# WPI-MMR/gym_solo

Measured on AMD Instinct MI355X. Metric: env-steps/s (whole node), 4096 Solo8 envs/GPU, 1/2/4/8 MI355X, higher is better.
Workload: dtype f64

## Files before the change

### gym_solo_amd/csrc/solo_engine.hip

```cpp
#include <hip/hip_runtime.h>

#include <cstdio>
#include <cstdlib>
#include <cstring>
#include <new>
#include <string>
#include <vector>

#ifndef SOLO_F64_PAIR_BUILD
#define SOLO_F64_PAIR_BUILD 1
#endif
#include "solo_wave_ops.h"
#include "solo_pgs_gfx950.h"
#include "solo_step_kernel.h"
#include "solo_launch.h"

namespace solo_engine_detail {

struct EngineBase {
  virtual ~EngineBase() {}
  virtual int set_program(const SoloProgram* p) = 0;
  virtual int reset(const uint8_t* mask, hipStream_t s) = 0;
  virtual int settle(hipStream_t s) = 0;
  virtual int set_targets(const void* a, hipStream_t s) = 0;
// ... 273 lines not shown
    if (int rc = check_flags(flags)) return rc;
    HIP_TRY(hipSetDevice(device));
    return launch((const T*)a, flags, s);
  }

  static constexpr int kWavesPerSimd = solo::kWavesPerSimd<T>;
  int resident_robots() const {
    hipDeviceProp_t p;
    const int cus = (hipGetDeviceProperties(&p, device) == hipSuccess && p.multiProcessorCount > 0) ? p.multiProcessorCount : 256;
    return cus * 4 * kWavesPerSimd;
  }
  int resident_cache = 0;
  solo::PlanInput plan_input(int k, uint32_t flags) {
    if (resident_cache == 0) resident_cache = resident_robots();
    return {n, sizeof(T), resident_cache, cfg.steps_per_launch, cfg.rollout_streams, cfg.migrate_steps, ctl_active(), sensing, k, flags,
            settling ? 1 : decimation, state_terms, act_on, wrench_on};
  }
  Plan make_plan(int k, uint32_t flags) { return solo::make_plan(plan_input(k, flags)); }
  int ensure_scratch(const Plan& p, uint32_t flags) {
    const bool records = solo::leaves_records(flags);
    if (records && p.S > traj_steps) {
      HIP_TRY(hipDeviceSynchronize());
      if (traj) { (void)hipFree(traj); traj = nullptr; traj_steps = 0; }
      HIP_TRY(hipMalloc((void**)&traj, solo::record_reals(n, p.S) * sizeof(T)));
      traj_steps = p.S;
      if (contact_traj) { (void)hipFree(contact_traj); contact_traj = nullptr; }
    }
    if (sensing && records && contact_traj == nullptr && traj_steps > 0) {
      HIP_TRY(hipDeviceSynchronize());
      HIP_TRY(hipMalloc((void**)&contact_traj, solo::foot_force_reals(n, traj_steps) * sizeof(T)));
      hparams.contact_traj = contact_traj;
// ... 10 lines not shown
    return SOLO_OK;
  }

  Args rollout_args(const void* a, int k, uint32_t flags, void* obs_out, void* reward_out, void* done_out) const {
    return Args{(const T*)a, a ? (long long)n * SOLO_NUM_JOINTS : 0, k, flags, (flags & SOLO_STEP_OBS) ? (T*)obs_out : nullptr,
                (flags & SOLO_STEP_REWARD) ? (T*)reward_out : nullptr, (flags & SOLO_STEP_DONE) ? (uint8_t*)done_out : nullptr};
  }

  int rollout(const void* a, int k, uint32_t flags, void* obs_out, void* reward_out, void* done_out, hipStream_t s) override {
    if (int rc = check_fault()) return rc;
    if (int rc = check_flags(flags)) return rc;
    if (k == 0) return SOLO_OK;
    if (!a || k < 0) { err = "rollout needs actions [K][N][12]"; return SOLO_ERR_INVALID_ARG; }
    const Plan plan = make_plan(k, flags);
    const Args args = rollout_args(a, k, flags, obs_out, reward_out, done_out);
    if (int rc = rollout_impl(plan, args, s, nullptr, nullptr)) return rc;
    if (!solo::tail_needs_copy<T>(plan, k, flags)) return SOLO_OK;
    if (args.obs_out)
      HIP_TRY(hipMemcpyAsync(obs, args.obs_out + (size_t)(k - 1) * n * obs_dim, (size_t)n * obs_dim * sizeof(T), hipMemcpyDeviceToDevice, s));
    if (args.reward_out)
      HIP_TRY(hipMemcpyAsync(reward, args.reward_out + (size_t)(k - 1) * n, (size_t)n * sizeof(T), hipMemcpyDeviceToDevice, s));
    if (args.done_out)
      HIP_TRY(hipMemcpyAsync(done, args.done_out + (size_t)(k - 1) * n, (size_t)n, hipMemcpyDeviceToDevice, s));
    return SOLO_OK;
  }

  int rollout_impl(const Plan& plan, const Args& args, hipStream_t s, hipEvent_t* t0, hipEvent_t* t1) {
    HIP_TRY(hipSetDevice(device));
    const int groups = plan.slices;
    if (int rc = ensure_scratch(plan, args.flags)) return rc;
// ... 23 lines not shown
    return SOLO_OK;
  }

  int enqueue(const Plan& plan, const Args& args, const solo::EngineBuffers<T>& wired, const solo::Launch& l, bool resid, hipStream_t s) {
    solo::KBuffers<T> b;
    solo::QueueInit q;
    if (!solo::wire_launch(plan, args, wired, l, &b, &q)) {
      err = "internal error: the migration queue of a launch does not fit its slice's region";
      return SOLO_ERR_INVALID_ARG;
    }
    if (q.ints > 0) {
      launch_flat(solo::solo_queue_init_kernel, q.ints, s, q.q, q.ints, q.lo, q.count, q.rings, q.steps, q.chunk, q.order);
      HIP_TRY(hipGetLastError());
    }
    const solo::KParams<T>* params_dev = dparams;
    solo::with_step_kernel<T>(solo::choose_kernel(sensing, ctl_active(), settling, resid, b.queue != nullptr, args.flags, decimation, state_terms, act_on, wrench_on),
                              [&](solo::StepKernel<T> k) { hipLaunchKernelGGL(k, dim3(l.count), dim3(64), 0, s, params_dev, b); });
    HIP_TRY(hipGetLastError());
    return SOLO_OK;
  }

  hipStream_t sub[kMaxStreams] = {};
  hipEvent_t ev_fork = nullptr, ev_join[kMaxStreams] = {};
  int ensure_streams(int groups) {
    if (!ev_fork) HIP_TRY(hipEventCreateWithFlags(&ev_fork, hipEventDisableTiming));
    for (int g = 0; g < groups; ++g) {
      if (!sub[g]) HIP_TRY(hipStreamCreateWithFlags(&sub[g], hipStreamNonBlocking));
      if (!ev_join[g]) HIP_TRY(hipEventCreateWithFlags(&ev_join[g], hipEventDisableTiming));
    }
    return SOLO_OK;
  }
// ... 11 lines not shown
    for (int g = 0; g < plan.slices; ++g) {
      float t = 0;
      HIP_TRY(hipEventElapsedTime(&t, e0[g], e1[g]));
      total += t;
    }
    *ms = total / plan.slices / plan.launches;
    return SOLO_OK;
  }

  int time_step(const void* a, uint32_t flags, int reps, hipStream_t s, double* ms) override {
    if (int rc = check_flags(flags)) return rc;
    if (reps <= 0 || !ms) { err = "reps must be positive"; return SOLO_ERR_INVALID_ARG; }
    HIP_TRY(hipSetDevice(device));
    const int S = cfg.steps_per_launch > 1 ? cfg.steps_per_launch : 1;
    Plan plan = make_plan(reps * S, flags);
    if (cfg.steps_per_launch == -1) {
      plan.S = 1; plan.launches = reps; plan.migrate = 0;
      if (cfg.rollout_streams == -1) plan.slices = 1;
    }
    return timed(plan, rollout_args(a, reps * S, flags, nullptr, nullptr, nullptr), s, ms);
  }

  int time_rollout(const void* a, int k, uint32_t flags, void* obs_out, void* reward_out, void* done_out, hipStream_t s, double* ms) override {
    if (int rc = check_flags(flags)) return rc;
    if (k <= 0 || !ms) { err = "num_steps must be positive"; return SOLO_ERR_INVALID_ARG; }
    HIP_TRY(hipSetDevice(device));
    return timed(make_plan(k, flags), rollout_args(a, k, flags, obs_out, reward_out, done_out), s, ms);
  }

  int reserve(int k, uint32_t flags) override {
    if (k <= 0) { err = "num_steps must be positive"; return SOLO_ERR_INVALID_ARG; }
    if (int rc = check_flags(flags)) return rc;
    HIP_TRY(hipSetDevice(device));
    return solo::for_each_geometry(plan_input(k, flags), k, [&](const Plan& p) {
      if (int rc = ensure_scratch(p, flags)) return rc;
      return p.slices > 1 ? ensure_streams(p.slices) : (int)SOLO_OK;
    });
  }

  int plan(int k, SoloLaunchPlan* out) override {
    if (k <= 0 || !out) { err = "num_steps must be positive"; return SOLO_ERR_INVALID_ARG; }
// ... 204 lines not shown
      const std::vector<T> ones((size_t)n * SOLO_ACTUATOR_WIDTH, T(1));
      HIP_TRY(hipMalloc((void**)&act_ones, ones.size() * sizeof(T)));
      HIP_TRY(hipMemcpy(act_ones, ones.data(), ones.size() * sizeof(T), hipMemcpyHostToDevice));
    }
    if (wrench == nullptr) {
      HIP_TRY(hipMalloc((void**)&wrench, cnt * sizeof(T)));
      hparams.wrench = wrench;
      HIP_TRY(hipMemcpy(dparams, &hparams, sizeof(hparams), hipMemcpyHostToDevice));
    }
    if ((const void*)wrench != per_env) HIP_TRY(hipMemcpy(wrench, h.data(), cnt * sizeof(T), hipMemcpyHostToDevice));
    wrench_on = true;
    return point_actuators();
  }

  std::string name;
  const char* kernel_name() override {
    name = solo::kernel_name(solo::choose_kernel(sensing, ctl_active(), false, cfg.solver_residual_threshold > 0, false, SOLO_STEP_ALL, decimation, state_terms, act_on, wrench_on), sizeof(T));
    return name.c_str();
  }
};

EngineBase* make_engine_f64(const SoloConfig& cfg, const SoloModel& model, int32_t num_envs, int32_t device_id, int* rc);
#ifndef SOLO_TU_F32
EngineBase* make_engine_f64(const SoloConfig& cfg, const SoloModel& model, int32_t num_envs, int32_t device_id, int* rc) {
  auto* e = new (std::nothrow) Engine<double>();
  *rc = e ? e->init(cfg, model, num_envs, device_id) : (int)SOLO_ERR_HIP;
  return e;
}
#endif

}

// ... 162 lines not shown
```

### gym_solo_amd/csrc/solo_kernel_params.h

```cpp
#pragma once

#include <cmath>
#include <cstdint>
#include <cstring>
#include <string>

#include "../../include/solo_engine.h"

namespace solo {

enum RowType : int32_t { ROW_IDLE = 0, ROW_MOTOR = 1, ROW_NORMAL = 2, ROW_TAN1 = 3, ROW_TAN2 = 4, ROW_LIMIT = 5 };
enum BodyKind : int32_t { BODY_BASE = 0, BODY_UPPER = 1, BODY_LOWER = 2 };

__host__ __device__ constexpr int motor_lane(int dof) { return 16 * (dof >> 1) + (dof & 1); }
__host__ __device__ constexpr int sphere_lane(int s) { return 16 * (s >> 2) + 2 + 3 * (s & 3); }

__host__ __device__ constexpr int leg_sum_entry(int e) {
  constexpr int Z = 10, N = 32;
  constexpr int b[27] = {0, 3, 1, 4, 5, 2,
                         Z, 8, 7 | N, 9,
                         8 | N, Z, 6, Z, 9,
                         7, 6 | N, Z, Z, Z, 9,
                         11, 12, 13, 14, 15, 16};
  constexpr int i[27] = {0, 1, 1, 2, 2, 2, 3, 3, 3, 3, 4, 4, 4, 4, 4, 5, 5, 5, 5, 5, 5, 0, 1, 2, 3, 4, 5};
// ... 129 lines not shown
  int32_t* term_count;
  double* stats;
  const T* terrain;
  const int32_t* order;
  int32_t* cost;
  T* warm;
  int32_t num_envs;
  uint32_t flags;
  int32_t env_base;
  int32_t count;
  int32_t steps;
  long long action_stride, done_stride;
  int32_t* queue;
  int32_t q_rings, q_chunk;
  int32_t* fault;
#ifdef SOLO_STAMPS
  int32_t stamp_row;
  unsigned long long* stamps;
  unsigned long long* acc;
#endif
};

inline int validate_model(const SoloModel& m, std::string* err) {
  auto fail = [&](const char* s) { if (err) *err = s; return (int)SOLO_ERR_UNSUPPORTED_MODEL; };
  for (int leg = 0; leg < 4; ++leg) {
    if (m.parent[2 * leg] != 0) return fail("HFE link must hang off the base");
    if (m.parent[2 * leg + 1] != 1 + 2 * leg) return fail("KFE link must hang off its HFE link");
  }
  for (int j = 0; j < SOLO_NUM_DOF; ++j)
    if (m.joint_axis[j][0] != 0.0 || m.joint_axis[j][1] != 1.0 || m.joint_axis[j][2] != 0.0)
// ... 165 lines not shown
```

### gym_solo_amd/csrc/solo_launch.h

```cpp
#pragma once

#include <string>

#include "solo_kernel_params.h"

namespace solo {

constexpr int kMaxStreams = 8;

struct Plan { int S, launches, slices, migrate; };

struct PlanInput {
  int n;
  size_t real_bytes;
  int resident;
  int32_t steps_per_launch, rollout_streams, migrate_steps;
  bool ctl_active, sensing;
  int k;
  uint32_t flags;
  int decimation = 1;
  bool state_terms = false;
  bool actuators = false;
  bool wrench = false;
};

inline Plan make_plan(const PlanInput& in) {
  const int n = in.n, k = in.k;
  const uint32_t flags = in.flags;
  const long long cap = ((1ll << 32) - 1) / ((long long)n * SOLO_STATE_STRIDE);
  const int decim = in.decimation > 1 ? in.decimation : 1;
  const int S_auto = 250 / decim > 1 ? 250 / decim : 1;
  long long want = in.steps_per_launch == -1 ? (k < S_auto ? k : S_auto) : (in.steps_per_launch > 1 ? in.steps_per_launch : 1);
  if (want > k && k > 0) want = k;
  Plan p;
  p.S = (int)(want < cap ? want : (cap > 1 ? cap : 1));
  if (p.S < 1) p.S = 1;
  p.launches = (k + p.S - 1) / p.S;
  const bool physics_only = flags == SOLO_STEP_PHYSICS;
  int streams = in.rollout_streams == -1 ? (p.launches > 1 ? 2 : 1) : in.rollout_streams;
  streams = streams < 1 ? 1 : (streams > kMaxStreams ? kMaxStreams : streams);
  p.migrate = 0;
#ifndef SOLO_STAMPS
  if (decim > 1 || in.state_terms || in.actuators || in.wrench) p.migrate = 0;
  else if (in.migrate_steps > 0) p.migrate = in.migrate_steps;
  else if (in.migrate_steps == -1 && !physics_only && (flags & SOLO_STEP_PHYSICS) && p.S >= 8 && !in.ctl_active && !in.sensing) {
    if (n > in.resident && in.real_bytes == 8) {
      if (p.launches == 1) p.migrate = (p.S + 1) / 2;
      else if (p.S >= 50) { p.migrate = 25; if (in.rollout_streams == -1) streams = 1; }
    }
  }
#endif
  p.slices = (streams > 1 && n >= 2 * streams) ? streams : 1;
  return p;
}

inline int max_slices(int n, int32_t rollout_streams) {
  const int streams = rollout_streams == -1 ? 2 : (rollout_streams < 1 ? 1 : (rollout_streams > kMaxStreams ? kMaxStreams : rollout_streams));
  return (streams > 1 && n >= 2 * streams) ? streams : 1;
}

inline int slice_begin(int n, int g, int groups) { return (int)((long long)n * g / groups); }

inline int queue_slots_per_robot(const Plan& p) {
  const int chunks = migration_chunks(p.S, p.migrate);
  return 1 + (chunks < 127 ? chunks : 127);
}

inline bool leaves_records(uint32_t flags) { return (flags & (SOLO_STEP_OBS | SOLO_STEP_REWARD)) != 0; }
inline size_t record_reals(int n, int steps) { return (size_t)steps * (size_t)n * SOLO_STATE_STRIDE; }
inline size_t foot_force_reals(int n, int steps) { return (size_t)steps * (size_t)n * 4; }
inline size_t queue_ints(int n, const Plan& p) {
  return p.migrate > 0 ? (size_t)kMaxStreams * kQueueHeader + (size_t)n * (size_t)queue_slots_per_robot(p) : 0;
}

template <class F>
inline int for_each_geometry(PlanInput in, int k, F&& f) {
  int last_S = -1, last_m = -1;
  for (int kk = 1; kk <= k; kk = (kk < 512 ? kk + 1 : (kk * 2 < k ? kk * 2 : (kk == k ? k + 1 : k)))) {
    in.k = kk;
    const Plan p = make_plan(in);
    if (p.S == last_S && p.migrate == last_m) continue;
    last_S = p.S; last_m = p.migrate;
    if (int rc = f(p)) return rc;
  }
  return 0;
}

enum KernelFamily : int { KERNEL_STEP = 0, KERNEL_CTL = 1, KERNEL_CONTACT = 2, KERNEL_DECIM = 3, KERNEL_TERM = 4, KERNEL_ACT = 5, KERNEL_PUSH = 6 };
struct KernelId {
  KernelFamily family;
  bool full, resid, migrate, ctl;
};

inline KernelId choose_kernel(bool sensing, bool ctl_active, bool settling, bool resid, bool has_queue, uint32_t flags, int decimation = 1,
                              bool state_terms = false, bool actuators = false, bool wrench = false) {
  const bool full = flags != SOLO_STEP_PHYSICS;
  if (wrench && !settling && (flags & SOLO_STEP_PHYSICS)) return {KERNEL_PUSH, full, false, false, ctl_active};
  if (actuators && !settling && ((flags & SOLO_STEP_PHYSICS) || (state_terms && (flags & SOLO_STEP_DONE)))) return {KERNEL_ACT, full, false, false, ctl_active};
  if (state_terms && !settling && (flags & (SOLO_STEP_PHYSICS | SOLO_STEP_DONE))) return {KERNEL_TERM, full, false, false, ctl_active};
  if (decimation > 1 && !settling && (flags & SOLO_STEP_PHYSICS)) return {KERNEL_DECIM, full, false, false, ctl_active};
  if (sensing && !settling) return {KERNEL_CONTACT, full, false, false, ctl_active};
  if (ctl_active && !settling) return {KERNEL_CTL, full, false, false, true};
  if (has_queue) return {KERNEL_STEP, true, resid, true, false};
  return {KERNEL_STEP, full, resid, false, false};
}

inline std::string kernel_name(const KernelId& id, size_t real_bytes) {
  const auto b = [](bool v) { return v ? ", true" : ", false"; };
  const std::string real = real_bytes == 4 ? "float" : "double";
  switch (id.family) {
    case KERNEL_CONTACT: return "solo_contact_kernel<" + real + b(id.full) + b(id.ctl) + ">";
    case KERNEL_CTL: return "solo_ctl_step_kernel<" + real + b(id.full) + ">";
    case KERNEL_DECIM: return "solo_decim_kernel<" + real + b(id.full) + b(id.ctl) + ">";
    case KERNEL_TERM: return "solo_term_kernel<" + real + b(id.full) + b(id.ctl) + ">";
    case KERNEL_ACT: return "solo_act_kernel<" + real + b(id.full) + b(id.ctl) + ">";
    case KERNEL_PUSH: return "solo_push_kernel<" + real + b(id.full) + b(id.ctl) + ">";
    default: return "solo_step_kernel<" + real + b(id.full) + b(id.resid) + b(id.migrate) + ">";
  }
}

template <typename T>
using StepKernel = void (*)(const KParams<T>*, KBuffers<T>);

template <typename T, class F>
inline void with_step_kernel(const KernelId& id, F&& f) {
  StepKernel<T> k;
  if (id.family == KERNEL_CONTACT) {
    if (id.ctl) k = !id.full ? solo_contact_kernel<T, false, true> : solo_contact_kernel<T, true, true>;
    else k = !id.full ? solo_contact_kernel<T, false, false> : solo_contact_kernel<T, true, false>;
  } else if (id.family == KERNEL_DECIM) {
    if (id.ctl) k = !id.full ? solo_decim_kernel<T, false, true> : solo_decim_kernel<T, true, true>;
    else k = !id.full ? solo_decim_kernel<T, false, false> : solo_decim_kernel<T, true, false>;
  } else if (id.family == KERNEL_TERM) {
    if (id.ctl) k = !id.full ? solo_term_kernel<T, false, true> : solo_term_kernel<T, true, true>;
    else k = !id.full ? solo_term_kernel<T, false, false> : solo_term_kernel<T, true, false>;
  } else if (id.family == KERNEL_ACT) {
    if (id.ctl) k = !id.full ? solo_act_kernel<T, false, true> : solo_act_kernel<T, true, true>;
    else k = !id.full ? solo_act_kernel<T, false, false> : solo_act_kernel<T, true, false>;
  } else if (id.family == KERNEL_PUSH) {
    if (id.ctl) k = !id.full ? solo_push_kernel<T, false, true> : solo_push_kernel<T, true, true>;
    else k = !id.full ? solo_push_kernel<T, false, false> : solo_push_kernel<T, true, false>;
  } else if (id.family == KERNEL_CTL) {
    k = !id.full ? solo_ctl_step_kernel<T, false> : solo_ctl_step_kernel<T, true>;
  } else if (id.migrate) {
    k = id.resid ? solo_step_kernel<T, true, true, true> : solo_step_kernel<T, true, false, true>;
  } else if (!id.full) {
    k = id.resid ? solo_step_kernel<T, false, true> : solo_step_kernel<T, false, false>;
  } else {
    k = id.resid ? solo_step_kernel<T, true, true> : solo_step_kernel<T, true, false>;
  }
  f(k);
}

template <typename T>
struct EngineBuffers {
  T *state, *snapshot, *targets, *params;
  T *obs, *reward;
  uint8_t* done;
// ... 17 lines not shown
template <typename T>
struct RolloutArgs {
  const T* act;
  long long act_stride;
  int k;
  uint32_t flags;
  T *obs_out, *reward_out;
  uint8_t* done_out;
};

struct Launch {
  int i, steps, lo, count, slice;
  bool final_chunk;
};

template <class F>
inline int for_each_launch(const Plan& plan, int n, int k, F&& f) {
  const int S = plan.S, groups = plan.slices;
  for (int i = 0; i < k; i += S)
    for (int g = 0; g < groups; ++g) {
      const int lo = slice_begin(n, g, groups), hi = slice_begin(n, g + 1, groups);
      if (int rc = f(Launch{i, (k - i < S) ? (k - i) : S, lo, hi - lo, g, i + S >= k})) return rc;
    }
  return 0;
}

struct QueueInit {
  int32_t* q;
  size_t ints;
  int lo, count, rings, steps, chunk;
  const int32_t* order;
};

template <typename T>
inline bool wire_launch(const Plan& plan, const RolloutArgs<T>& a, const EngineBuffers<T>& e, const Launch& l, KBuffers<T>* out, QueueInit* qi) {
  const int n = e.n, i = l.i, steps = l.steps;
  const uint32_t flags = a.flags;
  KBuffers<T>& b = *out;
  b.state = e.state; b.snapshot = e.snapshot; b.targets = e.targets; b.actions = a.act ? a.act + (size_t)i * a.act_stride : nullptr;
  b.params = e.params; b.traj = nullptr; b.obs_inline = b.reward_inline = nullptr; b.done = e.done; b.term_count = e.term_count;
  b.obs_rec = b.reward_rec = b.view_obs = b.view_reward = nullptr; b.view_done = nullptr; b.obs_rec_stride = b.reward_rec_stride = 0; b.obs_from = 0;
  b.stats = e.stats; b.terrain = e.terrain; b.order = e.order; b.cost = e.cost; b.num_envs = n; b.flags = flags;
  b.env_base = l.lo; b.count = l.count; b.steps = steps;
  b.action_stride = a.act_stride; b.done_stride = 0;
  b.queue = nullptr; b.q_rings = 1; b.q_chunk = 0;
  b.fault = e.fault;
  b.warm = e.warm;
#ifdef SOLO_STAMPS
  b.stamps = e.stamps;
#endif
  if (a.done_out) { b.done = a.done_out + (size_t)i * n; b.done_stride = n; }
  const bool want_obs = (flags & SOLO_STEP_OBS) != 0, want_reward = (flags & SOLO_STEP_REWARD) != 0;
  const bool inline_outputs = steps == 1 && (want_obs || want_reward) && kInlineOutputs<T, true>;
  if (inline_outputs) {
    if (want_obs) b.obs_inline = a.obs_out ? a.obs_out + (size_t)i * n * e.obs_dim : e.obs;
    if (want_reward) b.reward_inline = a.reward_out ? a.reward_out + (size_t)i * n : e.reward;
  } else if (want_obs || want_reward) {
    b.traj = e.traj + (size_t)l.lo * (size_t)e.traj_steps * SOLO_STATE_STRIDE;
    const bool tail_to_view = l.final_chunk;
    if (want_obs) {
      if (a.obs_out) { b.obs_rec = a.obs_out + (size_t)i * n * e.obs_dim; b.obs_rec_stride = (long long)n * e.obs_dim; if (tail_to_view) b.view_obs = e.obs; }
      else b.view_obs = e.obs;
// ... 9 lines not shown
    const int chunk = migration_chunk_steps(steps, plan.migrate);
    b.q_chunk = chunk;
    b.q_rings = migration_rings(l.count);
    b.queue = e.queue + (size_t)l.slice * kQueueHeader + (size_t)l.lo * (size_t)queue_slots_per_robot(plan);
    const size_t ints = migration_queue_ints(l.count, steps, chunk);
    if (ints > (size_t)kQueueHeader + (size_t)l.count * (size_t)queue_slots_per_robot(plan) ||
        (size_t)(b.queue - e.queue) + ints > e.queue_len)
      return false;
    *qi = QueueInit{b.queue, ints, l.lo, l.count, b.q_rings, steps, chunk, e.order};
  }
  return true;
}

template <typename T>
inline bool tail_needs_copy(const Plan& plan, int k, uint32_t flags) {
  const int last_steps = (k % plan.S == 0) ? plan.S : k % plan.S;
  return !leaves_records(flags) || (last_steps == 1 && kInlineOutputs<T, true>);
}

template <typename T>
inline void pack_control(const SoloConfig& cfg, const SoloControl& c, KParams<T>* P) {
  CtlConst<T>& k = P->ctl;
  k.mode = c.mode;
  for (int d = 0; d < SOLO_NUM_DOF; ++d) { k.kp[d] = (T)c.kp[d]; k.kd[d] = (T)c.kd[d]; }
  k.action_scale = (T)(c.mode == SOLO_CTRL_POSITION ? cfg.action_scale : c.action_scale);
  for (int j = 0; j < SOLO_NUM_JOINTS; ++j) k.reset_cmd[j] = (T)(c.mode == SOLO_CTRL_TORQUE ? 0.0 : cfg.settle_targets[j]);
}

template <typename T>
inline int validate_actuators(const T* host, int n, std::string* err) {
  for (size_t i = 0; i < (size_t)n * SOLO_ACTUATOR_WIDTH; ++i)
// ... 44 lines not shown
```

### gym_solo_amd/csrc/solo_step_body.h

```cpp
#pragma once

namespace solo {

template <typename T, bool kFull, bool kResid, bool kMigrate, bool kCtl, bool kContact, bool kDecim, bool kTerms, bool kAct = false, bool kPush = false>
__device__ __forceinline__ void step_body(const KParams<T>* Pin, const KBuffers<T>& Bin) {
  static_assert(!kTerms || kDecim, "the termination kernels run the substep loop");
  static_assert(!kAct || (kTerms && !kContact && !kResid && !kMigrate), "the actuator kernels are termination kernels: slot 25 of s_leg is theirs, and no robot migrates");
  static_assert(!kPush || kAct, "the push kernels are actuator kernels: their body plus the wrench");
  KBuffers<T> B = Bin;
  if (!kFull) B.flags = SOLO_STEP_PHYSICS;
  using R = Real<T>;
  __shared__ T s_state[SOLO_STATE_STRIDE];
  constexpr int kRS = ColumnBank<T>::kRowStride;
  constexpr int kRowsReals = kRowBlockReals<T>;
  constexpr int kGeoRows = SOLO_MAX_SPHERES + 1;
  __shared__ T s_blk[kRowsReals + kGeoRows * 4];
  static_assert(kRowsReals >= SOLO_MAX_REWARD_OPS * (kRowsReals / SOLO_MAX_REWARD_OPS < 32 ? kRowsReals / SOLO_MAX_REWARD_OPS : 32), "the output epilogue's scratch");
  T* const s_rowvec = s_blk;
  T (*const s_hext)[8] = ColumnBank<T>::kCompact ? nullptr : reinterpret_cast<T (*)[8]>(s_blk + 64 * kRS);
  __shared__ unsigned char s_rowleg[64];
  T (*const s_rowgeo)[4] = reinterpret_cast<T (*)[4]>(s_blk + kRowsReals);
  __shared__ int32_t s_rowtype[64];
  __shared__ T s_keep[32];
  __shared__ T s_leg[4][kLegSlots];
// ... 17 lines not shown
#pragma unroll
    for (int t = 0; t < SOLO_MAX_TERMS; ++t) r = r || solo_term_kind_reads_state(s_termtick[t]);
    return r;
  };
  const int lane0 = lane_id();
  const int slot = block_id() + B.env_base;
  if (slot >= B.num_envs) return;
  if (wave_cold_args(Bin)->num_envs != B.num_envs || wave_cold_args(Bin)->steps != B.steps) __builtin_trap();
  const int32_t* order = wave_cold_args(Bin)->order;
  int32_t* const queue = kMigrate ? wave_cold_args(Bin)->queue : nullptr;
  int env = 0, step_begin = 0, step_end = B.steps;
  bool last_chunk = true;
  int q_ring = 0, q_rings_left = 0, q_sweeps = 0, q_chunk_at = 0;
  int next_ticket = 0;
  bool have_next = false;
  if constexpr (!kMigrate) env = order != nullptr ? wave_uniform(order[slot]) : B.env_base + xcd_contiguous(block_id(), B.count);
  else {
    const int per_xcd = B.q_rings >= 8 ? B.q_rings >> 3 : 1;
    q_ring = B.q_rings >= 8 ? (wave_xcc_id() & 7) * per_xcd + (block_id() >> 3) % per_xcd : 0;
    q_rings_left = B.q_rings;
  }
#ifdef SOLO_STAMPS
  B.stamp_row = env;
#ifndef SOLO_STAMPS_LIGHT
  __shared__ unsigned long long s_acc[17];
  if (lane0 < 17) s_acc[lane0] = lane0 == 16 ? __builtin_amdgcn_s_memtime() : 0ull;
  B.acc = s_acc;
  wave_sync();
#endif
#endif
// ... 81 lines not shown
      if (ready >= 0) break;
      wave_backoff();
    }
    if (ready < 0) {
      if (lane0 == 0) { stats_add(&wave_cold_args(Bin)->stats[6], 1.0); if (wave_cold_args(Bin)->fault != nullptr) wave_fault_set(wave_cold_args(Bin)->fault); }
      break;
    }
    wave_acquire_device();
    env = B.env_base + (ready & 0xffffff);
    q_chunk_at = ready >> 24;
    step_begin = q_chunk_at * B.q_chunk;
    step_end = step_begin + B.q_chunk < B.steps ? step_begin + B.q_chunk : B.steps;
    last_chunk = step_end == B.steps;
  }
  const size_t rec = (size_t)env * SOLO_STATE_STRIDE;
  if constexpr (!ColumnBank<T>::kCompact) {
#pragma unroll
    for (int i = 0; i < 8; ++i) s_hext[lane0][i] = T(0);
  }
  if constexpr (!kMigrate) load_tables();
  T state_w = T(0);
  int count_w = 0;
  if constexpr (kMigrate) {
    if (lane0 < SOLO_STATE_STRIDE) state_w = wave_load_shared(wave_cold_args(Bin)->state + rec + lane0);
    if (lane0 < SOLO_MAX_TERMS) count_w = wave_atomic_load(wave_cold_args(Bin)->term_count + (size_t)env * SOLO_MAX_TERMS + lane0);
  } else {
    if (lane0 < SOLO_STATE_STRIDE) state_w = wave_cold_args(Bin)->state[rec + lane0];
    if (lane0 < SOLO_MAX_TERMS) count_w = wave_cold_args(Bin)->term_count[(size_t)env * SOLO_MAX_TERMS + lane0];
  }
  T foot_w = T(0);
  if constexpr (kContact) { if (lane0 < 4) foot_w = P0->contact[((size_t)env * SOLO_MAX_SPHERES + 4 * lane0 + 1) * SOLO_CONTACT_WIDTH + 3]; }
  const T mu = wave_cold_args(Bin)->params[(size_t)env * 4 + 0];
  const T mass_scale = wave_cold_args(Bin)->params[(size_t)env * 4 + 1];
  const T mu_base = P0->mu_base;
  T act_w = T(1);
  if constexpr (kAct) { if (lane0 < 3) act_w = P0->actuators[(size_t)env * SOLO_ACTUATOR_WIDTH + lane0]; }
  int hist_w = 0, prio_steps = 0;
  int prio_unit = 1;
  if constexpr (kDecim) prio_unit = wave_uniform(P0->decimation);
  if (B.steps == 1) {
    const int32_t* cost = wave_cold_args(Bin)->cost;
    if ((B.flags & SOLO_STEP_PHYSICS) && cost != nullptr) { hist_w = cost[env]; prio_steps = prio_unit; }
  }
  if constexpr (kMigrate) {
    if (lane0 == 0) hist_w = wave_atomic_load(queue + kQueueHeader + (env - B.env_base));
    hist_w = wave_readlane_int(hist_w, 0);
    prio_steps = step_begin;
  }
  {
    if constexpr (!kMigrate) store_tables();
    if (lane0 < SOLO_STATE_STRIDE) s_state[lane0] = state_w;
    if (lane0 < SOLO_MAX_TERMS) s_cnt[lane0] = count_w;
    if constexpr (sizeof(T) == 8) { if (lane0 == 0) { s_keep[27] = mu; s_keep[28] = mass_scale; } }
    if (lane0 == 0) s_keep[29] = mu_base;
    if constexpr (kContact) { if (lane0 < 4) s_leg[lane0][25] = foot_w; }
    if constexpr (kAct) {
      if (lane0 < 2) s_keep[30 + lane0] = act_w;
      const T act_kd = wave_readlane(act_w, SOLO_ACT_KD);
      if (lane0 < 4) s_leg[lane0][25] = act_kd;
    }
  }
  int prio_sweeps = wave_uniform(hist_w);
  const int hist_sweeps = kMigrate ? 0 : prio_sweeps;
  int prio_rot = (prio_steps + wave_slot_id()) % 3;
  if (prio_steps > 0) wave_set_priority_level(prio_sweeps > kPrioSweeps<T> * (kMigrate ? prio_steps : prio_unit) ? 3 : wave_slot_id() % 3);
  wave_sync();
  if constexpr (!kMigrate) make_term_tables();
  const bool may_restart = (B.flags & SOLO_STEP_DONE) && (B.flags & (SOLO_STEP_PHYSICS | SOLO_STEP_AUTO_RESET)) &&
                           wave_uniform(s_const.auto_reset) != 0;

  wave_sync();
#pragma unroll 1
  for (int step = step_begin; step < step_end; ++step) {
    const StepConst<T>& C = s_const;
    constexpr bool kLean = sizeof(T) == 8;
    int lane = kLean ? wave_fresh_lane() : wave_opaque_lane(lane0);
    const bool have_actions = kLean ? wave_opaque_bits((unsigned long long)B.actions) != 0ull : B.actions != nullptr;
    const T* const actions = have_actions ? B.actions : nullptr;
    const StepTables<T> tabs = {s_legc, s_rowtype, s_rowgeo};
    bool motor_lane = (s_rowtype[lane] & 15) == ROW_MOTOR;
    auto fetch_target = [&](int ln) -> T {
      const size_t tgt_at = (size_t)env * SOLO_NUM_JOINTS + (size_t)(3 * (ln >> 4) + (ln & 15));
// ... 118 lines not shown
        if (rt == ROW_TAN2) {
          T* const out = P0->contact + ((size_t)env * SOLO_MAX_SPHERES + sph) * SOLO_CONTACT_WIDTH;
          const T zr = T(wave_opaque_lane(0));
          out[0] = zr; out[1] = zr; out[2] = zr; out[3] = zr;
          if ((sph & 3) == 1) s_leg[sph >> 2][25] = zr;
        }
      }
      wave_sync();
      if (B.traj != nullptr && lane < 4)
        P0->contact_traj[((size_t)env * P0->contact_traj_steps + step) * 4 + lane] = s_leg[lane][25];
    }
    if (B.traj != nullptr) {
      const T ev = T((done ? kEventDone : 0) | (restart ? kEventRestart : 0) | fired_bits);
      const T word = s_state[lane & (SOLO_STATE_STRIDE - 1)];
      if (lane < SOLO_STATE_STRIDE)
        B.traj[(unsigned)((env - B.env_base) * B.steps + step) * (unsigned)SOLO_STATE_STRIDE + (unsigned)lane] = lane == SOLO_S_SPARE ? ev : word;
    }
    if constexpr (kInlineOutputs<T, kFull>) if (B.obs_inline != nullptr || B.reward_inline != nullptr) {
      const int n_obs = wave_uniform(C.num_obs), n_rops = wave_uniform(C.num_reward_ops);
      const ObsElemK<T> prog_obs = P0->obs[lane < n_obs ? lane : 0];
      const RewardInstrK<T> prog_reward = P0->reward[lane < n_rops ? lane : 0];
      const T angle = euler_component<T>(lane < 3 ? lane : 0, s_state[SOLO_S_QUAT], s_state[SOLO_S_QUAT + 1], s_state[SOLO_S_QUAT + 2], s_state[SOLO_S_QUAT + 3]);
      const T roll = wave_readlane(angle, 0), pitch = wave_readlane(angle, 1), yaw = wave_readlane(angle, 2);
      if (B.obs_inline != nullptr && lane < n_obs) {
        if constexpr (kContact) B.obs_inline[(size_t)env * n_obs + lane] = observation_value_foot<T>(prog_obs, s_state, roll, pitch, yaw, &s_leg[0][25], kLegSlots);
        else B.obs_inline[(size_t)env * n_obs + lane] = observation_value<T>(prog_obs, s_state, roll, pitch, yaw);
      }
      if (B.reward_inline != nullptr) {
        const RewardInstrK<T>& ri = prog_reward;
        T myval = reward_is_leaf(ri.op) ? reward_leaf<T>(ri, s_state, roll, pitch) : T(0);
        for (int i = 0; i < n_rops; ++i) {
// ... 35 lines not shown
    }
    SOLO_STAMP(B, 12);
    wave_sync();
  }
  SOLO_STAMP(B, 13);
  const int lane1 = sizeof(T) == 8 ? wave_fresh_lane() : wave_opaque_lane(lane0);
  if constexpr (kFull) if (B.traj != nullptr) {
    wave_fence_global();
    SOLO_STAMP_E(B, 1);
    const auto A = wave_cold_args(Bin);
    const int n_obs = wave_uniform(s_const.num_obs), n_rops = wave_uniform(s_const.num_reward_ops);
    constexpr int kPass = kRowsReals / SOLO_MAX_REWARD_OPS < 32 ? kRowsReals / SOLO_MAX_REWARD_OPS : 32;
    static_assert(kPass >= 16 && sizeof(T) * 32 >= (size_t)kPass, "the output epilogue's scratch");
    T* const val = s_blk;
    uint8_t* const ev_bytes = reinterpret_cast<uint8_t*>(s_keep);
    const T* const my_traj = B.traj + (size_t)(env - B.env_base) * (size_t)B.steps * SOLO_STATE_STRIDE;
    const bool want_reward = (B.flags & SOLO_STEP_REWARD) != 0;
    const bool bookkeeping = want_reward && (B.flags & SOLO_STEP_DONE) != 0;
    T* const obs_rec = A->obs_rec; T* const reward_rec = A->reward_rec;
    T* const view_obs = A->view_obs; T* const view_reward = A->view_reward; uint8_t* const view_done = A->view_done;
    const long long obs_stride = A->obs_rec_stride, reward_stride = A->reward_rec_stride;
    const int obs_from = A->obs_from;
    for (int base = step_begin; base < step_end; base += kPass) {
      const int k = base + lane1;
      if (lane1 < kPass && k < step_end) {
        const T* rec = my_traj + (size_t)k * SOLO_STATE_STRIDE;
        const bool last = k == B.steps - 1;
        const int ev = (int)rec[SOLO_S_SPARE];
        ev_bytes[lane1] = (uint8_t)ev;
        if (B.flags & SOLO_STEP_DONE) {
          if (B.done_stride != 0 || last) B.done[(size_t)k * B.done_stride + env] = (uint8_t)(ev & kEventDone);
          if (view_done != nullptr && last) view_done[env] = (uint8_t)(ev & kEventDone);
          if constexpr (kTerms) { if (last && (!kAct || state_program())) P0->term_fired[env] = (uint8_t)(ev >> 2); }
        }
        SOLO_STAMP_E(B, 2);
        T roll, pitch, yaw;
        euler_from_quat<T>(rec[SOLO_S_QUAT], rec[SOLO_S_QUAT + 1], rec[SOLO_S_QUAT + 2], rec[SOLO_S_QUAT + 3], &roll, &pitch, &yaw);
        SOLO_STAMP_E(B, 3);
        if (B.flags & SOLO_STEP_OBS) {
          T* o_rec = (obs_rec != nullptr && k >= obs_from) ? obs_rec + (size_t)k * obs_stride + (size_t)env * n_obs : nullptr;
          T* o_view = (view_obs != nullptr && last) ? view_obs + (size_t)env * n_obs : nullptr;
// ... 13 lines not shown
          if (view_reward != nullptr && last) view_reward[env] = rv;
        }
        SOLO_STAMP_E(B, 5);
      }
      wave_sync();
      SOLO_STAMP_E(B, 6);
      if (bookkeeping && lane1 == 0) {
        const int cnt = step_end - base < kPass ? step_end - base : kPass;
        accumulate_returns<T>(s_state, ev_bytes, 1, val + (size_t)(n_rops - 1) * kPass, 1, cnt, SOLO_STATS_ROW,
                              [](double* p, double x) { stats_add(p, x); });
      }
      wave_sync();
      SOLO_STAMP_E(B, 7);
    }
  }
  if ((B.flags & SOLO_STEP_DONE) && lane1 < SOLO_MAX_TERMS) {
    if constexpr (kMigrate) wave_atomic_store(wave_cold_args(Bin)->term_count + (size_t)env * SOLO_MAX_TERMS + lane1, s_cnt[lane1]);
    else wave_cold_args(Bin)->term_count[(size_t)env * SOLO_MAX_TERMS + lane1] = s_cnt[lane1];
  }
  if ((B.flags & SOLO_STEP_PHYSICS) && lane1 == 0 && last_chunk) { int32_t* cost = wave_cold_args(Bin)->cost; if (cost != nullptr) cost[env] = prio_sweeps - hist_sweeps; }
  const bool own_returns = (B.flags & SOLO_STEP_REWARD) && (B.flags & SOLO_STEP_DONE) &&
                           (B.traj != nullptr || (kInlineOutputs<T, kFull> && B.reward_inline != nullptr));
  if (lane1 < (own_returns ? SOLO_S_SPARE : SOLO_S_RETURN)) {
    if constexpr (kMigrate) wave_store_shared(wave_cold_args(Bin)->state + rec + lane1, s_state[lane1]);
    else wave_cold_args(Bin)->state[rec + lane1] = s_state[lane1];
  }
  SOLO_STAMP(B, 14);
#if defined(SOLO_STAMPS) && !defined(SOLO_STAMPS_LIGHT)
  wave_sync();
  if (lane1 < 16) B.stamps[(size_t)env * 32 + 16 + lane1] = s_acc[lane1];
#endif
  if constexpr (kMigrate) {
    const int chunks = migration_chunks(B.steps, B.q_chunk), ring_len = (B.count / B.q_rings) * chunks;
    int at = 0, nt = 0;
    if (lane1 == 0) {
      if (!last_chunk) {
        wave_atomic_store(queue + kQueueHeader + (env - B.env_base), prio_sweeps);
        at = wave_atomic_add(queue + q_ring * 32 + 16, 1);
      }
      nt = wave_atomic_add(queue + q_ring * 32, 1);
    }
    wave_release_device();
    if (!last_chunk && lane1 == 0)
      wave_atomic_store(queue + kQueueHeader + (size_t)B.count + (size_t)q_ring * ring_len + at, (env - B.env_base) | ((q_chunk_at + 1) << 24));
    next_ticket = wave_readlane_int(nt, 0);
    have_next = true;
  }
  if constexpr (kMigrate) wave_sync();
  } while (kMigrate);
#undef SOLO_STATS_ROW
}

}
```

### gym_solo_amd/csrc/solo_step_kernel.h

```cpp
#pragma once

#include "solo_kernel_params.h"
#include "solo_outputs.h"

#if defined(SOLO_STAMPS) && defined(SOLO_STAMPS_LIGHT)
#define SOLO_STAMP(B, i)                                                                          \
  do {                                                                                            \
    if (((i) == 0 || (i) == 14) && solo::lane_id() == 0)                                          \
      (B).stamps[(size_t)(B).stamp_row * 32 + (i)] = __builtin_amdgcn_s_memrealtime();         \
  } while (0)
#elif defined(SOLO_STAMPS)
#ifdef SOLO_STAMPS_EPILOGUE
#define SOLO_STAMP_ON(i) ((i) == 0 || (i) >= 13)
#define SOLO_STAMP_E(B, i) SOLO_STAMP_AT(B, i)
#else
#define SOLO_STAMP_ON(i) true
#endif
#define SOLO_STAMP(B, i) do { if (SOLO_STAMP_ON(i)) SOLO_STAMP_AT(B, i); } while (0)
#define SOLO_STAMP_AT(B, i)                                                                       \
  do {                                                                                            \
    if (solo::lane_id() == 0) {                                                                   \
      const unsigned long long t_ = __builtin_amdgcn_s_memtime();                                 \
      (B).stamps[(size_t)(B).stamp_row * 32 + (i)] = t_;                                            \
      (B).acc[(i)] += t_ - (B).acc[16];                                                           \
// ... 958 lines not shown
__global__ __launch_bounds__(64, kWavesPerSimd<T>) void solo_term_kernel(const KParams<T>* __restrict__ Pin, KBuffers<T> Bin) {
  step_body<T, kFull, false, false, kCtl, false, true, true>(Pin, Bin);
}

template <typename T, bool kFull, bool kCtl>
__global__ __launch_bounds__(64, kWavesPerSimd<T>) void solo_act_kernel(const KParams<T>* __restrict__ Pin, KBuffers<T> Bin) {
  step_body<T, kFull, false, false, kCtl, false, true, true, true>(Pin, Bin);
}

template <typename T, bool kFull, bool kCtl>
__global__ __launch_bounds__(64, kWavesPerSimd<T>) void solo_push_kernel(const KParams<T>* __restrict__ Pin, KBuffers<T> Bin) {
  step_body<T, kFull, false, false, kCtl, false, true, true, true, true>(Pin, Bin);
}

template <typename T>
__global__ void solo_contact_zero_kernel(T* __restrict__ contact, const uint8_t* __restrict__ mask, int num_envs) {
  const int i = blockIdx.x * blockDim.x + threadIdx.x;
  const int env = i / (SOLO_MAX_SPHERES * SOLO_CONTACT_WIDTH);
  if (env >= num_envs) return;
  if (mask != nullptr && mask[env] == 0) return;
  contact[i] = T(0);
}

static __global__ void solo_queue_init_kernel(int32_t* __restrict__ q, size_t ints, int env_base, int n, int rings, int steps, int chunk,
                                       const int32_t* __restrict__ order) {
  const size_t i = (size_t)blockIdx.x * blockDim.x + threadIdx.x;
  if (i < ints) migration_queue_init(q, i, env_base, n, rings, steps, chunk, order);
}

template <typename T>
// ... 43 lines not shown
```

Before: 200.0 million.

## Fuse multiple rollout launches into one segmented roll kernel

```diff
diff --git a/gym_solo_amd/csrc/solo_engine.hip b/gym_solo_amd/csrc/solo_engine.hip
--- a/gym_solo_amd/csrc/solo_engine.hip
+++ b/gym_solo_amd/csrc/solo_engine.hip
@@ -311,7 +311,7 @@
   solo::PlanInput plan_input(int k, uint32_t flags) {
     if (resident_cache == 0) resident_cache = resident_robots();
     return {n, sizeof(T), resident_cache, cfg.steps_per_launch, cfg.rollout_streams, cfg.migrate_steps, ctl_active(), sensing, k, flags,
-            settling ? 1 : decimation, state_terms, act_on, wrench_on};
+            settling ? 1 : decimation, state_terms, act_on, wrench_on, !settling && !(cfg.solver_residual_threshold > 0)};
   }
   Plan make_plan(int k, uint32_t flags) { return solo::make_plan(plan_input(k, flags)); }
   int ensure_scratch(const Plan& p, uint32_t flags) {
@@ -352,6 +352,7 @@
     if (!a || k < 0) { err = "rollout needs actions [K][N][12]"; return SOLO_ERR_INVALID_ARG; }
     const Plan plan = make_plan(k, flags);
     const Args args = rollout_args(a, k, flags, obs_out, reward_out, done_out);
+    rolled = false;
     if (int rc = rollout_impl(plan, args, s, nullptr, nullptr)) return rc;
     if (!solo::tail_needs_copy<T>(plan, k, flags)) return SOLO_OK;
     if (args.obs_out)
@@ -405,7 +406,9 @@
       HIP_TRY(hipGetLastError());
     }
     const solo::KParams<T>* params_dev = dparams;
-    solo::with_step_kernel<T>(solo::choose_kernel(sensing, ctl_active(), settling, resid, b.queue != nullptr, args.flags, decimation, state_terms, act_on, wrench_on),
+    const bool segmented = b.seg_steps > 0;
+    if (segmented) rolled = true;
+    solo::with_step_kernel<T>(solo::choose_kernel(sensing, ctl_active(), settling, resid, b.queue != nullptr, args.flags, decimation, state_terms, act_on, wrench_on, segmented),
                               [&](solo::StepKernel<T> k) { hipLaunchKernelGGL(k, dim3(l.count), dim3(64), 0, s, params_dev, b); });
     HIP_TRY(hipGetLastError());
     return SOLO_OK;
@@ -447,10 +450,12 @@
     HIP_TRY(hipSetDevice(device));
     const int S = cfg.steps_per_launch > 1 ? cfg.steps_per_launch : 1;
     Plan plan = make_plan(reps * S, flags);
+    plan.fuse = 0;
     if (cfg.steps_per_launch == -1) {
       plan.S = 1; plan.launches = reps; plan.migrate = 0;
       if (cfg.rollout_streams == -1) plan.slices = 1;
     }
+    rolled = false;
     return timed(plan, rollout_args(a, reps * S, flags, nullptr, nullptr, nullptr), s, ms);
   }
 
@@ -458,6 +463,7 @@
     if (int rc = check_flags(flags)) return rc;
     if (k <= 0 || !ms) { err = "num_steps must be positive"; return SOLO_ERR_INVALID_ARG; }
     HIP_TRY(hipSetDevice(device));
+    rolled = false;
     return timed(make_plan(k, flags), rollout_args(a, k, flags, obs_out, reward_out, done_out), s, ms);
   }
 
@@ -692,8 +698,9 @@
   }
 
   std::string name;
+  bool rolled = false;
   const char* kernel_name() override {
-    name = solo::kernel_name(solo::choose_kernel(sensing, ctl_active(), false, cfg.solver_residual_threshold > 0, false, SOLO_STEP_ALL, decimation, state_terms, act_on, wrench_on), sizeof(T));
+    name = solo::kernel_name(solo::choose_kernel(sensing, ctl_active(), false, cfg.solver_residual_threshold > 0, false, SOLO_STEP_ALL, decimation, state_terms, act_on, wrench_on, rolled), sizeof(T));
     return name.c_str();
   }
 };
diff --git a/gym_solo_amd/csrc/solo_kernel_params.h b/gym_solo_amd/csrc/solo_kernel_params.h
--- a/gym_solo_amd/csrc/solo_kernel_params.h
+++ b/gym_solo_amd/csrc/solo_kernel_params.h
@@ -167,6 +167,7 @@
   int32_t* queue;
   int32_t q_rings, q_chunk;
   int32_t* fault;
+  int32_t seg_steps;
 #ifdef SOLO_STAMPS
   int32_t stamp_row;
   unsigned long long* stamps;
diff --git a/gym_solo_amd/csrc/solo_launch.h b/gym_solo_amd/csrc/solo_launch.h
--- a/gym_solo_amd/csrc/solo_launch.h
+++ b/gym_solo_amd/csrc/solo_launch.h
@@ -8,7 +8,8 @@
 
 constexpr int kMaxStreams = 8;
 
-struct Plan { int S, launches, slices, migrate; };
+constexpr int kMaxFusedSegments = 16;
+struct Plan { int S, launches, slices, migrate; int fuse = 0; };
 
 struct PlanInput {
   int n;
@@ -22,7 +23,10 @@
   bool state_terms = false;
   bool actuators = false;
   bool wrench = false;
-};
+  bool fuse = false;
+};
+
+inline bool leaves_records(uint32_t flags);
 
 inline Plan make_plan(const PlanInput& in) {
   const int n = in.n, k = in.k;
@@ -51,6 +55,12 @@
   }
 #endif
   p.slices = (streams > 1 && n >= 2 * streams) ? streams : 1;
+  p.fuse = 0;
+#if !defined(SOLO_STAMPS) || defined(SOLO_STAMPS_LIGHT)
+  if (in.fuse && p.launches > 1 && p.S > 1 && p.migrate == 0 && !in.ctl_active && !in.sensing && decim == 1 && !in.state_terms &&
+      !in.actuators && !in.wrench && leaves_records(flags) && (flags & SOLO_STEP_PHYSICS))
+    p.fuse = p.launches < kMaxFusedSegments ? p.launches : kMaxFusedSegments;
+#endif
   return p;
 }
 
@@ -75,25 +85,25 @@
 
 template <class F>
 inline int for_each_geometry(PlanInput in, int k, F&& f) {
-  int last_S = -1, last_m = -1;
+  int last_S = -1, last_m = -1, last_slices = -1, last_fuse = -1;
   for (int kk = 1; kk <= k; kk = (kk < 512 ? kk + 1 : (kk * 2 < k ? kk * 2 : (kk == k ? k + 1 : k)))) {
     in.k = kk;
     const Plan p = make_plan(in);
-    if (p.S == last_S && p.migrate == last_m) continue;
-    last_S = p.S; last_m = p.migrate;
+    if (p.S == last_S && p.migrate == last_m && p.slices == last_slices && p.fuse == last_fuse) continue;
+    last_S = p.S; last_m = p.migrate; last_slices = p.slices; last_fuse = p.fuse;
     if (int rc = f(p)) return rc;
   }
   return 0;
 }
 
-enum KernelFamily : int { KERNEL_STEP = 0, KERNEL_CTL = 1, KERNEL_CONTACT = 2, KERNEL_DECIM = 3, KERNEL_TERM = 4, KERNEL_ACT = 5, KERNEL_PUSH = 6 };
+enum KernelFamily : int { KERNEL_STEP = 0, KERNEL_CTL = 1, KERNEL_CONTACT = 2, KERNEL_DECIM = 3, KERNEL_TERM = 4, KERNEL_ACT = 5, KERNEL_PUSH = 6, KERNEL_ROLL = 7 };
 struct KernelId {
   KernelFamily family;
   bool full, resid, migrate, ctl;
 };
 
 inline KernelId choose_kernel(bool sensing, bool ctl_active, bool settling, bool resid, bool has_queue, uint32_t flags, int decimation = 1,
-                              bool state_terms = false, bool actuators = false, bool wrench = false) {
+                              bool state_terms = false, bool actuators = false, bool wrench = false, bool segmented = false) {
   const bool full = flags != SOLO_STEP_PHYSICS;
   if (wrench && !settling && (flags & SOLO_STEP_PHYSICS)) return {KERNEL_PUSH, full, false, false, ctl_active};
   if (actuators && !settling && ((flags & SOLO_STEP_PHYSICS) || (state_terms && (flags & SOLO_STEP_DONE)))) return {KERNEL_ACT, full, false, false, ctl_active};
@@ -102,6 +112,7 @@
   if (sensing && !settling) return {KERNEL_CONTACT, full, false, false, ctl_active};
   if (ctl_active && !settling) return {KERNEL_CTL, full, false, false, true};
   if (has_queue) return {KERNEL_STEP, true, resid, true, false};
+  if (segmented && full && !resid) return {KERNEL_ROLL, true, false, false, false};
   return {KERNEL_STEP, full, resid, false, false};
 }
 
@@ -115,6 +126,7 @@
     case KERNEL_TERM: return "solo_term_kernel<" + real + b(id.full) + b(id.ctl) + ">";
     case KERNEL_ACT: return "solo_act_kernel<" + real + b(id.full) + b(id.ctl) + ">";
     case KERNEL_PUSH: return "solo_push_kernel<" + real + b(id.full) + b(id.ctl) + ">";
+    case KERNEL_ROLL: return "solo_roll_kernel<" + real + ">";
     default: return "solo_step_kernel<" + real + b(id.full) + b(id.resid) + b(id.migrate) + ">";
   }
 }
@@ -142,6 +154,8 @@
     else k = !id.full ? solo_push_kernel<T, false, false> : solo_push_kernel<T, true, false>;
   } else if (id.family == KERNEL_CTL) {
     k = !id.full ? solo_ctl_step_kernel<T, false> : solo_ctl_step_kernel<T, true>;
+  } else if (id.family == KERNEL_ROLL) {
+    k = solo_roll_kernel<T>;
   } else if (id.migrate) {
     k = id.resid ? solo_step_kernel<T, true, true, true> : solo_step_kernel<T, true, false, true>;
   } else if (!id.full) {
@@ -189,9 +203,11 @@
   bool final_chunk;
 };
 
+inline int launch_span(const Plan& plan) { return plan.fuse > 0 ? plan.fuse * plan.S : plan.S; }
+
 template <class F>
 inline int for_each_launch(const Plan& plan, int n, int k, F&& f) {
-  const int S = plan.S, groups = plan.slices;
+  const int S = launch_span(plan), groups = plan.slices;
   for (int i = 0; i < k; i += S)
     for (int g = 0; g < groups; ++g) {
       const int lo = slice_begin(n, g, groups), hi = slice_begin(n, g + 1, groups);
@@ -221,6 +237,7 @@
   b.queue = nullptr; b.q_rings = 1; b.q_chunk = 0;
   b.fault = e.fault;
   b.warm = e.warm;
+  b.seg_steps = steps > plan.S ? plan.S : 0;
 #ifdef SOLO_STAMPS
   b.stamps = e.stamps;
 #endif
@@ -260,7 +277,8 @@
 
 template <typename T>
 inline bool tail_needs_copy(const Plan& plan, int k, uint32_t flags) {
-  const int last_steps = (k % plan.S == 0) ? plan.S : k % plan.S;
+  const int span = launch_span(plan);
+  const int last_steps = (k % span == 0) ? span : k % span;
   return !leaves_records(flags) || (last_steps == 1 && kInlineOutputs<T, true>);
 }
 
diff --git a/gym_solo_amd/csrc/solo_step_body.h b/gym_solo_amd/csrc/solo_step_body.h
--- a/gym_solo_amd/csrc/solo_step_body.h
+++ b/gym_solo_amd/csrc/solo_step_body.h
@@ -2,11 +2,12 @@
 
 namespace solo {
 
-template <typename T, bool kFull, bool kResid, bool kMigrate, bool kCtl, bool kContact, bool kDecim, bool kTerms, bool kAct = false, bool kPush = false>
+template <typename T, bool kFull, bool kResid, bool kMigrate, bool kCtl, bool kContact, bool kDecim, bool kTerms, bool kAct = false, bool kPush = false, bool kSegments = false>
 __device__ __forceinline__ void step_body(const KParams<T>* Pin, const KBuffers<T>& Bin) {
   static_assert(!kTerms || kDecim, "the termination kernels run the substep loop");
   static_assert(!kAct || (kTerms && !kContact && !kResid && !kMigrate), "the actuator kernels are termination kernels: slot 25 of s_leg is theirs, and no robot migrates");
   static_assert(!kPush || kAct, "the push kernels are actuator kernels: their body plus the wrench");
+  static_assert(!kSegments || (kFull && !kResid && !kMigrate && !kCtl && !kContact && !kDecim && !kTerms && !kAct && !kPush), "the segmented kernel is the full position-control step: every other family needs its own register check");
   KBuffers<T> B = Bin;
   if (!kFull) B.flags = SOLO_STEP_PHYSICS;
   using R = Real<T>;
@@ -55,6 +56,13 @@
   int q_ring = 0, q_rings_left = 0, q_sweeps = 0, q_chunk_at = 0;
   int next_ticket = 0;
   bool have_next = false;
+  int seg_len = B.steps, carry_sweeps = 0, carry_steps = 0;
+  if constexpr (kSegments) {
+    const int seg = wave_cold_args(Bin)->seg_steps;
+    if (seg > 0 && seg < B.steps) seg_len = seg;
+    step_end = seg_len;
+    last_chunk = step_end == B.steps;
+  }
   if constexpr (!kMigrate) env = order != nullptr ? wave_uniform(order[slot]) : B.env_base + xcd_contiguous(block_id(), B.count);
   else {
     const int per_xcd = B.q_rings >= 8 ? B.q_rings >> 3 : 1;
@@ -166,17 +174,18 @@
     last_chunk = step_end == B.steps;
   }
   const size_t rec = (size_t)env * SOLO_STATE_STRIDE;
+  const bool first_seg = !kSegments || step_begin == 0;
   if constexpr (!ColumnBank<T>::kCompact) {
 #pragma unroll
     for (int i = 0; i < 8; ++i) s_hext[lane0][i] = T(0);
   }
-  if constexpr (!kMigrate) load_tables();
+  if constexpr (!kMigrate) { if (first_seg) load_tables(); }
   T state_w = T(0);
   int count_w = 0;
   if constexpr (kMigrate) {
     if (lane0 < SOLO_STATE_STRIDE) state_w = wave_load_shared(wave_cold_args(Bin)->state + rec + lane0);
     if (lane0 < SOLO_MAX_TERMS) count_w = wave_atomic_load(wave_cold_args(Bin)->term_count + (size_t)env * SOLO_MAX_TERMS + lane0);
-  } else {
+  } else if (first_seg) {
     if (lane0 < SOLO_STATE_STRIDE) state_w = wave_cold_args(Bin)->state[rec + lane0];
     if (lane0 < SOLO_MAX_TERMS) count_w = wave_cold_args(Bin)->term_count[(size_t)env * SOLO_MAX_TERMS + lane0];
   }
@@ -199,10 +208,13 @@
     hist_w = wave_readlane_int(hist_w, 0);
     prio_steps = step_begin;
   }
+  if constexpr (kSegments) { if (!first_seg) { hist_w = carry_sweeps; prio_steps = carry_steps; } }
   {
-    if constexpr (!kMigrate) store_tables();
-    if (lane0 < SOLO_STATE_STRIDE) s_state[lane0] = state_w;
-    if (lane0 < SOLO_MAX_TERMS) s_cnt[lane0] = count_w;
+    if constexpr (!kMigrate) { if (first_seg) store_tables(); }
+    if (first_seg) {
+      if (lane0 < SOLO_STATE_STRIDE) s_state[lane0] = state_w;
+      if (lane0 < SOLO_MAX_TERMS) s_cnt[lane0] = count_w;
+    }
     if constexpr (sizeof(T) == 8) { if (lane0 == 0) { s_keep[27] = mu; s_keep[28] = mass_scale; } }
     if (lane0 == 0) s_keep[29] = mu_base;
     if constexpr (kContact) { if (lane0 < 4) s_leg[lane0][25] = foot_w; }
@@ -215,9 +227,9 @@
   int prio_sweeps = wave_uniform(hist_w);
   const int hist_sweeps = kMigrate ? 0 : prio_sweeps;
   int prio_rot = (prio_steps + wave_slot_id()) % 3;
-  if (prio_steps > 0) wave_set_priority_level(prio_sweeps > kPrioSweeps<T> * (kMigrate ? prio_steps : prio_unit) ? 3 : wave_slot_id() % 3);
+  if (prio_steps > 0 && first_seg) wave_set_priority_level(prio_sweeps > kPrioSweeps<T> * (kMigrate ? prio_steps : prio_unit) ? 3 : wave_slot_id() % 3);
   wave_sync();
-  if constexpr (!kMigrate) make_term_tables();
+  if constexpr (!kMigrate) { if (first_seg) make_term_tables(); }
   const bool may_restart = (B.flags & SOLO_STEP_DONE) && (B.flags & (SOLO_STEP_PHYSICS | SOLO_STEP_AUTO_RESET)) &&
                            wave_uniform(s_const.auto_reset) != 0;
 
@@ -366,7 +378,7 @@
       const T ev = T((done ? kEventDone : 0) | (restart ? kEventRestart : 0) | fired_bits);
       const T word = s_state[lane & (SOLO_STATE_STRIDE - 1)];
       if (lane < SOLO_STATE_STRIDE)
-        B.traj[(unsigned)((env - B.env_base) * B.steps + step) * (unsigned)SOLO_STATE_STRIDE + (unsigned)lane] = lane == SOLO_S_SPARE ? ev : word;
+        B.traj[(unsigned)(kSegments ? (env - B.env_base) * seg_len + (step - step_begin) : (env - B.env_base) * B.steps + step) * (unsigned)SOLO_STATE_STRIDE + (unsigned)lane] = lane == SOLO_S_SPARE ? ev : word;
     }
     if constexpr (kInlineOutputs<T, kFull>) if (B.obs_inline != nullptr || B.reward_inline != nullptr) {
       const int n_obs = wave_uniform(C.num_obs), n_rops = wave_uniform(C.num_reward_ops);
@@ -432,7 +444,7 @@
     static_assert(kPass >= 16 && sizeof(T) * 32 >= (size_t)kPass, "the output epilogue's scratch");
     T* const val = s_blk;
     uint8_t* const ev_bytes = reinterpret_cast<uint8_t*>(s_keep);
-    const T* const my_traj = B.traj + (size_t)(env - B.env_base) * (size_t)B.steps * SOLO_STATE_STRIDE;
+    const T* const my_traj = B.traj + (size_t)(env - B.env_base) * (size_t)(kSegments ? seg_len : B.steps) * SOLO_STATE_STRIDE;
     const bool want_reward = (B.flags & SOLO_STEP_REWARD) != 0;
     const bool bookkeeping = want_reward && (B.flags & SOLO_STEP_DONE) != 0;
     T* const obs_rec = A->obs_rec; T* const reward_rec = A->reward_rec;
@@ -442,7 +454,7 @@
     for (int base = step_begin; base < step_end; base += kPass) {
       const int k = base + lane1;
       if (lane1 < kPass && k < step_end) {
-        const T* rec = my_traj + (size_t)k * SOLO_STATE_STRIDE;
+        const T* rec = my_traj + (size_t)(kSegments ? k - step_begin : k) * SOLO_STATE_STRIDE;
         const bool last = k == B.steps - 1;
         const int ev = (int)rec[SOLO_S_SPARE];
         ev_bytes[lane1] = (uint8_t)ev;
@@ -486,14 +498,14 @@
       SOLO_STAMP_E(B, 7);
     }
   }
-  if ((B.flags & SOLO_STEP_DONE) && lane1 < SOLO_MAX_TERMS) {
+  if ((B.flags & SOLO_STEP_DONE) && lane1 < SOLO_MAX_TERMS && (!kSegments || last_chunk)) {
     if constexpr (kMigrate) wave_atomic_store(wave_cold_args(Bin)->term_count + (size_t)env * SOLO_MAX_TERMS + lane1, s_cnt[lane1]);
     else wave_cold_args(Bin)->term_count[(size_t)env * SOLO_MAX_TERMS + lane1] = s_cnt[lane1];
   }
   if ((B.flags & SOLO_STEP_PHYSICS) && lane1 == 0 && last_chunk) { int32_t* cost = wave_cold_args(Bin)->cost; if (cost != nullptr) cost[env] = prio_sweeps - hist_sweeps; }
   const bool own_returns = (B.flags & SOLO_STEP_REWARD) && (B.flags & SOLO_STEP_DONE) &&
                            (B.traj != nullptr || (kInlineOutputs<T, kFull> && B.reward_inline != nullptr));
-  if (lane1 < (own_returns ? SOLO_S_SPARE : SOLO_S_RETURN)) {
+  if (lane1 < (own_returns ? SOLO_S_SPARE : SOLO_S_RETURN) && (!kSegments || last_chunk)) {
     if constexpr (kMigrate) wave_store_shared(wave_cold_args(Bin)->state + rec + lane1, s_state[lane1]);
     else wave_cold_args(Bin)->state[rec + lane1] = s_state[lane1];
   }
@@ -519,7 +531,15 @@
     have_next = true;
   }
   if constexpr (kMigrate) wave_sync();
-  } while (kMigrate);
+  if constexpr (kSegments) {
+    if (last_chunk) break;
+    wave_fence_global();
+    carry_sweeps = prio_sweeps; carry_steps = prio_steps;
+    step_begin += seg_len;
+    step_end = step_begin + seg_len < B.steps ? step_begin + seg_len : B.steps;
+    last_chunk = step_end == B.steps;
+  }
+  } while (kMigrate || kSegments);
 #undef SOLO_STATS_ROW
 }
 
diff --git a/gym_solo_amd/csrc/solo_step_kernel.h b/gym_solo_amd/csrc/solo_step_kernel.h
--- a/gym_solo_amd/csrc/solo_step_kernel.h
+++ b/gym_solo_amd/csrc/solo_step_kernel.h
@@ -996,6 +996,11 @@
 }
 
 template <typename T>
+__global__ __launch_bounds__(64, kWavesPerSimd<T>) void solo_roll_kernel(const KParams<T>* __restrict__ Pin, KBuffers<T> Bin) {
+  step_body<T, true, false, false, false, false, false, false, false, false, true>(Pin, Bin);
+}
+
+template <typename T>
 __global__ void solo_contact_zero_kernel(T* __restrict__ contact, const uint8_t* __restrict__ mask, int num_envs) {
   const int i = blockIdx.x * blockDim.x + threadIdx.x;
   const int env = i / (SOLO_MAX_SPHERES * SOLO_CONTACT_WIDTH);
```

New measurement: 206.3 million, median of 6. +3.1%, better.
